# LasseWolter/laughter-detection-icsi

Hardware: AMD Instinct MI355X
Metric: 1 s@16 kHz segments/sec (featurize+ResNet fwd/bwd) (higher is better)
Workload: dtype f32 (64->64 and 32->32 convolutions: f16x2 split operands with per-tile power-of-two scales, f32 accumulate; error vs float64 within 1.5x of the exact-f32 kernels'); 1 GPU; BASELINE configs[2]: end-to-end featurize (HIP fbank 44 mel) + ResNetBigger resnet_base fwd/bwd + clip + Adam, random labels, dropout 0.5; global_batch=512, parallelism=dp1, overlap_wgrad=False, overlap_wgrad_small=True, bf16x3_convs=True, f16x2_convs=True, relu_bits=True, virtual_a1=True

## Files before the change

### include/lad_hip.h

```cpp
#ifndef LAD_HIP_H
#define LAD_HIP_H

#include <stdint.h>

#ifdef __cplusplus
extern "C" {
#endif

#define LAD_VERSION 100

enum lad_status {
    LAD_OK = 0,
    LAD_ERR_INVALID = -1,
    LAD_ERR_HIP = -2,
    LAD_ERR_NOMEM = -3,
    LAD_NOT_COVERED = 1
};

int lad_version(void);
const char *lad_last_error(void);

enum lad_pad_mode {
    LAD_PAD_KALDI_MIRROR = 0,
    LAD_PAD_CENTER_REFLECT = 1,
// ... 132 lines not shown

int lad_stem_fwd(const float *feat, const float *weight, float *out, float *stat_partials, int64_t batch, int32_t H,
                 int32_t W, int32_t cout, void *stream);
int lad_stem_fwd_eval(const float *feat, const float *weight, const float *scale, const float *shift, float *out,
                      int64_t batch, int32_t H, int32_t W, int32_t cout, int64_t frame_stride, int64_t frames_avail,
                      void *stream);
int64_t lad_stem_moments_workspace_doubles(void);
int64_t lad_stem_moments_doubles(void);
int lad_stem_bn_stats(const float *feat, const float *weight, const float *gamma, const float *beta, float *running_mean,
                      float *running_var, float momentum, float *coef, double *moments, double *workspace, int64_t batch, int32_t H,
                      int32_t W, int32_t cout, void *stream);
int64_t lad_stem_bwd_onepass_workspace_floats(void);
int lad_stem_bwd_onepass(const float *feat, const float *weight, const float *dy, const float *coef, const float *gamma,
                         const double *moments, float *workspace, float *dw, float *dgamma, float *dbeta, int64_t batch, int32_t H,
                         int32_t W, int32_t cout, void *stream);
int64_t lad_stem_wgrad_workspace_floats(void);
int lad_stem_wgrad(const float *feat, const float *dout, float *workspace, float *dw, int64_t batch, int32_t H,
                   int32_t W, int32_t cout, void *stream);
int lad_stem_wgrad_bn(const float *feat, const float *dy, const float *x, const float *weight, const float *coef,
                      const float *bcoef, float *workspace, float *dw, int64_t batch, int32_t H, int32_t W, int32_t cout,
                      void *stream);
int64_t lad_stem_bn_bwd_groups(int64_t batch, int32_t H, int32_t W);
int lad_stem_bn_bwd_sums(const float *feat, const float *weight, const float *dy, const float *coef, float *partials,
                         int64_t batch, int32_t H, int32_t W, int32_t cout, void *stream);

int lad_bn_finalize(float *stat_partials, int64_t n_tiles, int32_t channels, int64_t count, const float *gamma,
                    const float *beta, float *running_mean, float *running_var, float momentum, float *coef,
                    void *stream);
int lad_bn_finalize_pair(float *stat_partials_a, float *stat_partials_b, int64_t n_tiles, int32_t channels, int64_t count,
                         const float *gamma_a, const float *beta_a, float *running_mean_a, float *running_var_a, float *coef_a,
                         const float *gamma_b, const float *beta_b, float *running_mean_b, float *running_var_b, float *coef_b,
                         float momentum, void *stream);
int lad_bn_act(const float *x, const float *coef, const float *res, const float *res_coef, float *y, int64_t batch,
               int32_t H, int32_t W, int32_t channels, int32_t relu, void *stream);
int64_t lad_bn_bwd_workspace_floats(int32_t channels);
int lad_bn_bwd(const float *dy, const float *y, const float *x, const float *coef, const float *gamma,
               const float *xs, const float *scoef, const float *sgamma, float *dx, float *aux, float *dgamma,
               float *dbeta, float *dsgamma, float *dsbeta, float *workspace, float *bcoef, float *pre_partials,
               int64_t pre_tiles, int64_t batch, int32_t H, int32_t W, int32_t channels, int32_t relu, int32_t mode,
               void *stream);
int lad_bn_act_bits(const float *x, const float *coef, const float *res, const float *res_coef, float *y,
                    uint64_t *y_bits, int64_t batch, int32_t H, int32_t W, int32_t channels, void *stream);
int lad_bn_bwd_bits(const float *dy, const uint64_t *y_bits, const float *x, const float *coef, const float *gamma,
                    float *dx, float *dgamma, float *dbeta, float *workspace, float *bcoef, float *pre_partials,
                    int64_t pre_tiles, int64_t batch, int32_t H, int32_t W, int32_t channels, void *stream);
int lad_conv_fwd_bnstat(const float *in, const float *wt, const float *addend, float *out, float *stat_partials,
                        const float *bn_x, const float *bn_y, const float *bn_coef, int64_t batch, int32_t H, int32_t W,
                        int32_t cin, int32_t cout, int32_t taps, void *stream);

int lad_pool_fwd(const float *x, float *pooled, int64_t batch, int32_t H, int32_t W, int32_t channels, void *stream);
int lad_pool_bwd(const float *dpooled, float *dx, int64_t batch, int32_t H, int32_t W, int32_t channels, void *stream);
int64_t lad_head_workspace_floats(int64_t batch, int32_t F);
int lad_head_fwd_train(const float *const *params, const float *pooled, int64_t batch, int32_t F, const float *drop1,
                       const float *drop2, const int32_t *labels, float momentum, float *h, float *stats,
                       float *probs, float *metrics, void *stream);
int lad_head_fwd_train_rng(const float *const *params, const float *pooled, int64_t batch, int32_t F, float *drop1, float *drop2, float keep,
                           uint64_t seed, int64_t *rng_counter, int64_t *nbt, int32_t n_nbt, const int32_t *labels, float momentum,
// ... 63 lines not shown
```

### laughter-detection-icsi_amd/_hip.py

```python
import ctypes
import os

import torch

_HERE = os.path.dirname(os.path.abspath(__file__))
LIB_PATH = os.environ.get("LAD_HIP_LIB") or os.path.join(_HERE, "liblad_hip.so")

c_void_p = ctypes.c_void_p
c_int = ctypes.c_int
c_i64 = ctypes.c_int64
c_float = ctypes.c_float
c_double = ctypes.c_double
c_i32 = ctypes.c_int32
c_float_p = ctypes.POINTER(ctypes.c_float)


class LadHipError(RuntimeError):
    pass


class FbankCfg(ctypes.Structure):
    _fields_ = [("n_fft", ctypes.c_int32), ("frame_len", ctypes.c_int32), ("hop", ctypes.c_int32),
                ("n_mels", ctypes.c_int32), ("n_mfcc", ctypes.c_int32), ("pad_mode", ctypes.c_int32),
                ("log_mode", ctypes.c_int32), ("remove_dc", ctypes.c_int32), ("preemph", ctypes.c_float),
# ... 67 lines not shown
    "lad_conv_wgrad": (c_int, [c_void_p] * 5 + [c_i64, c_i32, c_i32, c_i32, c_i32, c_i32, c_void_p]),
    "lad_stem_fwd": (c_int, [c_void_p] * 4 + [c_i64, c_i32, c_i32, c_i32, c_void_p]),
    "lad_stem_fwd_eval": (c_int, [c_void_p] * 5 + [c_i64, c_i32, c_i32, c_i32, c_i64, c_i64, c_void_p]),
    "lad_stem_wgrad_workspace_floats": (c_i64, []),
    "lad_stem_wgrad": (c_int, [c_void_p] * 4 + [c_i64, c_i32, c_i32, c_i32, c_void_p]),
    "lad_stem_wgrad_bn": (c_int, [c_void_p] * 8 + [c_i64, c_i32, c_i32, c_i32, c_void_p]),
    "lad_stem_bn_bwd_groups": (c_i64, [c_i64, c_i32, c_i32]),
    "lad_stem_bn_bwd_sums": (c_int, [c_void_p] * 5 + [c_i64, c_i32, c_i32, c_i32, c_void_p]),
    "lad_bn_finalize": (c_int, [c_void_p, c_i64, c_i32, c_i64, c_void_p, c_void_p, c_void_p, c_void_p, c_float,
                                c_void_p, c_void_p]),
    "lad_stem_moments_workspace_doubles": (c_i64, []),
    "lad_stem_moments_doubles": (c_i64, []),
    "lad_stem_bn_stats": (c_int, [c_void_p] * 6 + [c_float] + [c_void_p] * 3 + [c_i64, c_i32, c_i32, c_i32, c_void_p]),
    "lad_stem_bwd_onepass_workspace_floats": (c_i64, []),
    "lad_stem_bwd_onepass": (c_int, [c_void_p] * 10 + [c_i64, c_i32, c_i32, c_i32, c_void_p]),
    "lad_bn_finalize_pair": (c_int, [c_void_p, c_void_p, c_i64, c_i32, c_i64] + [c_void_p] * 10 + [c_float, c_void_p]),
    "lad_bn_act": (c_int, [c_void_p] * 5 + [c_i64, c_i32, c_i32, c_i32, c_i32, c_void_p]),
    "lad_bn_bwd_workspace_floats": (c_i64, [c_i32]),
    "lad_bn_act_bits": (c_int, [c_void_p] * 6 + [c_i64, c_i32, c_i32, c_i32, c_void_p]),
    "lad_bn_bwd_bits": (c_int, [c_void_p] * 11 + [c_i64, c_i64, c_i32, c_i32, c_i32, c_void_p]),
    "lad_bn_bwd": (c_int, [c_void_p] * 17 + [c_i64, c_i64, c_i32, c_i32, c_i32, c_i32, c_i32, c_void_p]),
    "lad_conv_fwd_bnstat": (c_int, [c_void_p] * 8 + [c_i64, c_i32, c_i32, c_i32, c_i32, c_i32, c_void_p]),
    "lad_pool_fwd": (c_int, [c_void_p, c_void_p, c_i64, c_i32, c_i32, c_i32, c_void_p]),
    "lad_pool_bwd": (c_int, [c_void_p, c_void_p, c_i64, c_i32, c_i32, c_i32, c_void_p]),
    "lad_head_workspace_floats": (c_i64, [c_i64, c_i32]),
    "lad_head_fwd_train": (c_int, [c_void_p, c_void_p, c_i64, c_i32, c_void_p, c_void_p, c_void_p, c_float,
                                   c_void_p, c_void_p, c_void_p, c_void_p, c_void_p]),
    "lad_head_fwd_train_rng": (c_int, [c_void_p, c_void_p, c_i64, c_i32, c_void_p, c_void_p, c_float, ctypes.c_uint64, c_void_p, c_void_p, c_i32,
                                       c_void_p, c_float, c_void_p, c_void_p, c_void_p, c_void_p, c_void_p]),
    "lad_head_fwd_eval": (c_int, [c_void_p, c_void_p, c_i64, c_i32, c_void_p, c_void_p]),
    "lad_bce_metrics": (c_int, [c_void_p, c_void_p, c_i64, c_void_p, c_void_p]),
    "lad_head_bwd": (c_int, [c_void_p] * 7 + [c_i64, c_i32] + [c_void_p] * 6),
    "lad_f16_packed_weight_halfs": (c_i64, [c_i32, c_i32, c_i32]),
    "lad_f16_pack_weights": (c_int, [c_void_p, c_i32, c_i32, c_i32, c_void_p, c_void_p]),
# ... 67 lines not shown
```

### laughter-detection-icsi_amd/csrc/bn.hip

```cpp
#include "lad_common.h"
#include "lad_device.h"
#include "lad_bn_math.h"

namespace {
using namespace lad;

constexpr float BN_EPS = 1e-5f;
constexpr int THREADS = 256;

struct FinSet {
    const float *partials, *gamma, *beta;
    float *running_mean, *running_var, *coef;
};
struct FinSets {
    FinSet s[2];
};
__global__ void bn_finalize_kernel(FinSets sets, int64_t n_tiles, int C, double count, float momentum) {
    const FinSet f = sets.s[blockIdx.y];
    const float *__restrict__ partials = f.partials;
    float *__restrict__ coef = f.coef;
    const int c = blockIdx.x;
    double s1 = 0.0, s2 = 0.0;
    int64_t t = threadIdx.x;
    const int64_t bd = blockDim.x;
// ... 218 lines not shown
                    const float4 rr = res[idx];
                    o.x += rr.x; o.y += rr.y; o.z += rr.z; o.w += rr.w;
                } else if (RES == 2) {
                    const float4 rr = res[idx];
                    o.x += fmaf(rr.x, rs.x, rh.x); o.y += fmaf(rr.y, rs.y, rh.y);
                    o.z += fmaf(rr.z, rs.z, rh.z); o.w += fmaf(rr.w, rs.w, rh.w);
                }
                if (relu) {
                    o.x = fmaxf(o.x, 0.f); o.y = fmaxf(o.y, 0.f); o.z = fmaxf(o.z, 0.f); o.w = fmaxf(o.w, 0.f);
                }
            }
            y[idx] = o;
            if (BITS) {
                const unsigned long long word = pack_sign_bits(o, threadIdx.x & 63);
                if ((threadIdx.x & 15) == 0) bits[idx >> 4] = word;
            }
        }
    }
}

template <int C, bool SHORT>
__global__ __launch_bounds__(THREADS) void bn_bwd_reduce_kernel(const float4 *__restrict__ dy, const float4 *__restrict__ y,
                                                                const float4 *__restrict__ x, const float *__restrict__ coef,
                                                                const float4 *__restrict__ xs, const float *__restrict__ scoef,
                                                                float *__restrict__ partials, int64_t rows, int relu,
                                                                const unsigned long long *__restrict__ bits) {
    constexpr int C4 = C / 4;
    constexpr int RP = THREADS / C4;
    constexpr int K = SHORT ? 3 : 2;
    const int c4 = threadIdx.x % C4, rp = threadIdx.x / C4;
// ... 285 lines not shown
}
}

extern "C" int lad_bn_act(const float *x, const float *coef, const float *res, const float *res_coef, float *y,
                          int64_t batch, int32_t H, int32_t W, int32_t channels, int32_t relu, void *stream) {
    return bn_act_impl(x, coef, res, res_coef, y, nullptr, batch, H, W, channels, relu, stream, "lad_bn_act");
}

extern "C" int lad_bn_act_bits(const float *x, const float *coef, const float *res, const float *res_coef, float *y,
                               uint64_t *y_bits, int64_t batch, int32_t H, int32_t W, int32_t channels, void *stream) {
    using namespace lad;
    LAD_REQUIRE(y_bits, "lad_bn_act_bits: null sign-bit buffer");
    return bn_act_impl(x, coef, res, res_coef, y, (unsigned long long *)y_bits, batch, H, W, channels, 1, stream, "lad_bn_act_bits");
}

extern "C" int64_t lad_bn_bwd_workspace_floats(int32_t channels) { return (int64_t)BWD_GROUPS * 3 * channels; }

namespace {
int bn_bwd_impl(const float *dy, const float *y, const unsigned long long *bits, const float *x, const float *coef, const float *gamma,
                const float *xs, const float *scoef, const float *sgamma, float *dx, float *aux,
                float *dgamma, float *dbeta, float *dsgamma, float *dsbeta, float *workspace, float *bcoef,
                float *pre_partials, int64_t pre_tiles, int64_t batch, int32_t H, int32_t W, int32_t channels,
                int32_t relu, int32_t mode, void *stream) {
    using namespace lad;
    LAD_REQUIRE(relu != 3 || (bits && channels == 64), "lad_bn_bwd_bits: sign bits are kept for 64-channel activations only");
    LAD_REQUIRE(dy && coef && gamma && dgamma && dbeta && workspace && bcoef, "lad_bn_bwd: null buffer");
    LAD_REQUIRE(x || (pre_partials && !dx), "lad_bn_bwd: x may only be omitted when the sums are given and nothing is applied");
    LAD_REQUIRE(dx || mode == 0, "lad_bn_bwd: dx may only be omitted (sums and coefficients only) in mode 0");
    LAD_REQUIRE(relu >= 0 && relu <= 3, "lad_bn_bwd: relu must be 0 (none), 1 (mask from y), 2 (mask recomputed from x) or 3 (sign bits: lad_bn_bwd_bits)");
    LAD_REQUIRE(relu != 1 || y, "lad_bn_bwd: relu = 1 needs y");
// ... 82 lines not shown
```

### laughter-detection-icsi_amd/csrc/lad_stem_taps.h

```cpp
#pragma once
#include "lad_device.h"

namespace lad {

constexpr int STEM_TM = 128;
constexpr int TAPW = 12;
__device__ __forceinline__ void fill_taps(const float *__restrict__ feat, const Geom &g, int H, int W, int64_t q0,
                                          int64_t frame_stride, int64_t frames_avail, float *tap_s ) {
    const int r = threadIdx.x;
    if (r < STEM_TM) {
        const int64_t q = q0 + r;
        float v[9];
#pragma unroll
        for (int t = 0; t < 9; ++t) v[t] = 0.0f;
        float flag = 0.0f;
        if (q < g.body) {
            const int64_t b = q / g.img;
            const int rr = (int)(q - b * g.img);
            const int yp = rr / g.Wp, xp = rr - yp * g.Wp;
            if (yp >= 1 && xp >= 1) {
                flag = 1.0f;
                const int y = yp - 1, x = xp - 1;
                const int64_t f0 = b * frame_stride;
#pragma unroll
                for (int ky = 0; ky < 3; ++ky)
#pragma unroll
                    for (int kx = 0; kx < 3; ++kx) {
                        const int yy = y + ky - 1, xx = x + kx - 1;
                        const bool ok = yy >= 0 && yy < H && xx >= 0 && xx < W && (f0 + yy) < frames_avail;
                        v[ky * 3 + kx] = ok ? feat[(f0 + yy) * W + xx] : 0.0f;
                    }
            }
        }
        float4 *dst = reinterpret_cast<float4 *>(tap_s + r * TAPW);
        dst[0] = make_float4(v[0], v[1], v[2], v[3]);
        dst[1] = make_float4(v[4], v[5], v[6], v[7]);
        dst[2] = make_float4(v[8], flag, 0.f, 0.f);
    }
}
__device__ __forceinline__ bool read_taps(const float *tap_s, int r, float (&v)[9]) {
    const float4 *src = reinterpret_cast<const float4 *>(tap_s + r * TAPW);
    const float4 a = src[0], b = src[1], c = src[2];
    v[0] = a.x; v[1] = a.y; v[2] = a.z; v[3] = a.w; v[4] = b.x; v[5] = b.y; v[6] = b.z; v[7] = b.w; v[8] = c.x;
    return c.y != 0.0f;
}


}
```

### laughter-detection-icsi_amd/csrc/stem.hip

```cpp
#include "lad_common.h"
#include "lad_device.h"
#include "lad_stem_taps.h"
#include "lad_bn_math.h"

namespace {
using namespace lad;

constexpr int THREADS = 256;
constexpr int TM = lad::STEM_TM;
constexpr int COUT = 64;
constexpr int CQ = COUT / 4;
constexpr int RL = THREADS / CQ;
constexpr int MAX_GROUPS = 1536;

template <bool STORE>
__global__ __launch_bounds__(THREADS) void stem_fwd_kernel(const float *__restrict__ feat, const float *__restrict__ w ,
                                                           float *__restrict__ out, float *__restrict__ partials, Geom g,
                                                           int H, int W) {
    const int tid = threadIdx.x, cq = tid % CQ, rl = tid / CQ;
    float wr[4][9];
#pragma unroll
    for (int c = 0; c < 4; ++c)
#pragma unroll
        for (int t = 0; t < 9; ++t) wr[c][t] = w[(cq * 4 + c) * 9 + t];
// ... 34 lines not shown
            const int k = tid / COUT, c = tid - k * COUT;
            float s = 0.f;
#pragma unroll
            for (int p = 0; p < RL; ++p) s += red[p][k][c];
            partials[((int64_t)blockIdx.x * 2 + k) * COUT + c] = s;
        }
    }
}

__global__ __launch_bounds__(THREADS) void stem_fwd_eval_kernel(const float *__restrict__ feat, const float *__restrict__ w,
                                                                const float *__restrict__ scale, const float *__restrict__ shift,
                                                                float *__restrict__ out, Geom g, int H, int W,
                                                                int64_t frame_stride, int64_t frames_avail) {
    const int tid = threadIdx.x, cq = tid % CQ, rl = tid / CQ;
    float wr[4][9];
#pragma unroll
    for (int c = 0; c < 4; ++c)
#pragma unroll
        for (int t = 0; t < 9; ++t) wr[c][t] = w[(cq * 4 + c) * 9 + t];
    const float4 sc = *reinterpret_cast<const float4 *>(scale + cq * 4);
    const float4 sh = *reinterpret_cast<const float4 *>(shift + cq * 4);
    const int64_t q0 = (int64_t)blockIdx.x * TM;
    __shared__ __attribute__((aligned(16))) float tap_s[TM * TAPW];
    fill_taps(feat, g, H, W, q0, frame_stride, frames_avail, tap_s);
    __syncthreads();
    for (int r = rl; r < TM; r += RL) {
        const int64_t q = q0 + r;
        if (q >= g.rows) break;
        float4 o = make_float4(0.f, 0.f, 0.f, 0.f);
        float v[9];
        if (read_taps(tap_s, r, v)) {
            float acc[4] = {0, 0, 0, 0};
#pragma unroll
            for (int t = 0; t < 9; ++t)
#pragma unroll
                for (int c = 0; c < 4; ++c) acc[c] = fmaf(v[t], wr[c][t], acc[c]);
            o = make_float4(fmaxf(fmaf(acc[0], sc.x, sh.x), 0.f), fmaxf(fmaf(acc[1], sc.y, sh.y), 0.f),
                            fmaxf(fmaf(acc[2], sc.z, sh.z), 0.f), fmaxf(fmaf(acc[3], sc.w, sh.w), 0.f));
        }
        *reinterpret_cast<float4 *>(out + q * COUT + cq * 4) = o;
    }
}

template <int MODE>
__global__ __launch_bounds__(THREADS) void stem_wgrad_kernel(const float *__restrict__ feat, const float *__restrict__ dout,
                                                             const float *__restrict__ x, const float *__restrict__ w,
                                                             const float *__restrict__ coef,
                                                             const float *__restrict__ bcoef, float *__restrict__ slabs,
                                                             Geom g, int H, int W, int64_t n_tiles) {
    const int tid = threadIdx.x, cq = tid % CQ, rl = tid / CQ;
    float acc[4][9];
#pragma unroll
    for (int c = 0; c < 4; ++c)
#pragma unroll
// ... 288 lines not shown
        coef[0 * COUT + c] = scale;
        coef[1 * COUT + c] = beta[c] - (float)mean * scale;
        coef[2 * COUT + c] = (float)mean;
        coef[3 * COUT + c] = invstd;
        coef[4 * COUT + c] = (float)(mean - (double)(float)mean);
        coef[5 * COUT + c] = (float)(invstd_d - (double)invstd);
        if (running_mean != nullptr) {
            const double unbiased = count > 1.0 ? var * count / (count - 1.0) : var;
            running_mean[c] = (1.0f - momentum) * running_mean[c] + momentum * (float)mean;
            running_var[c] = (1.0f - momentum) * running_var[c] + momentum * (float)unbiased;
        }
    }
}

constexpr int BWD1_COLS = COUT * 9 + 2 * COUT;
__global__ __launch_bounds__(THREADS) void stem_bwd_onepass_kernel(const float *__restrict__ feat, const float *__restrict__ w,
                                                                   const float *__restrict__ dy, const float *__restrict__ coef,
                                                                   const double *__restrict__ mom, float *__restrict__ slabs, Geom g, int H,
                                                                   int W, int64_t n_tiles) {
    const int tid = threadIdx.x, cq = tid % CQ, rl = tid / CQ;
    float acc[4][9];
#pragma unroll
    for (int c = 0; c < 4; ++c)
#pragma unroll
        for (int t = 0; t < 9; ++t) acc[c][t] = 0.f;
    float wr[4][9];
#pragma unroll
    for (int c = 0; c < 4; ++c)
#pragma unroll
        for (int t = 0; t < 9; ++t) wr[c][t] = w[(cq * 4 + c) * 9 + t];
    const float4 fsc = *reinterpret_cast<const float4 *>(coef + cq * 4);
    const float4 fsh = *reinterpret_cast<const float4 *>(coef + COUT + cq * 4);
    const Norm4 nm = load_norm(coef, COUT, cq * 4);
    const float m = (float)mom[MOM_N];
    float4 a0 = make_float4(0.f, 0.f, 0.f, 0.f), a1 = a0;
    __shared__ __attribute__((aligned(16))) float tap_s[TM * TAPW];
    constexpr int NR = TM / RL;
    for (int64_t tile = blockIdx.x; tile < n_tiles; tile += gridDim.x) {
        const int64_t q0 = tile * TM;
        float4 dv[NR];
#pragma unroll
        for (int k = 0; k < NR; ++k) {
            const int64_t q = q0 + rl + k * RL;
            dv[k] = q < g.rows ? *reinterpret_cast<const float4 *>(dy + q * COUT + cq * 4) : make_float4(0.f, 0.f, 0.f, 0.f);
        }
        __syncthreads();
        fill_taps(feat, g, H, W, q0, H, (int64_t)1 << 62, tap_s);
        __syncthreads();
#pragma unroll
        for (int k = 0; k < NR; ++k) {
            const int r = rl + k * RL;
            const int64_t q = q0 + r;
            if (q >= g.rows) break;
            float v[9];
            if (read_taps(tap_s, r, v)) {
                float xa[4] = {0, 0, 0, 0};
#pragma unroll
                for (int t = 0; t < 9; ++t)
#pragma unroll
                    for (int c = 0; c < 4; ++c) xa[c] = fmaf(v[t], wr[c][t], xa[c]);
                const float4 xv = make_float4(xa[0], xa[1], xa[2], xa[3]);
                const float4 d = mask_from_x(dv[k], xv, fsc, fsh);
                const float4 xh = xhat4(xv, nm);
                a0.x += d.x; a0.y += d.y; a0.z += d.z; a0.w += d.w;
                a1.x = fmaf(d.x, xh.x, a1.x); a1.y = fmaf(d.y, xh.y, a1.y); a1.z = fmaf(d.z, xh.z, a1.z); a1.w = fmaf(d.w, xh.w, a1.w);
                const float dd[4] = {d.x, d.y, d.z, d.w};
#pragma unroll
                for (int t = 0; t < 9; ++t) {
                    const float gt = v[t] - m;
#pragma unroll
                    for (int c = 0; c < 4; ++c) acc[c][t] = fmaf(gt, dd[c], acc[c][t]);
                }
            }
        }
    }
    __shared__ float red[RL][BWD1_COLS];
#pragma unroll
    for (int c = 0; c < 4; ++c)
#pragma unroll
        for (int t = 0; t < 9; ++t) red[rl][(cq * 4 + c) * 9 + t] = acc[c][t];
    *reinterpret_cast<float4 *>(&red[rl][COUT * 9 + cq * 4]) = a0;
    *reinterpret_cast<float4 *>(&red[rl][COUT * 10 + cq * 4]) = a1;
    __syncthreads();
    for (int e = tid; e < BWD1_COLS; e += THREADS) {
        float sacc = 0.f;
#pragma unroll
        for (int p = 0; p < RL; ++p) sacc += red[p][e];
        slabs[(int64_t)blockIdx.x * BWD1_COLS + e] = sacc;
// ... 159 lines not shown
    LAD_REQUIRE(cout == COUT && batch >= 1 && H >= 1 && W >= 1, "lad_stem_bn_stats: bad arguments");
    const int groups = (int)std::min<int64_t>(MOM_GROUPS, batch);
    const size_t lds = std::max<size_t>((size_t)(H + 2) * (W + 2) * sizeof(float), (size_t)18 * MOM_THREADS * sizeof(double));
    LAD_REQUIRE(lds <= 60 * 1024, "lad_stem_bn_stats: an image of %d x %d does not fit the workgroup's LDS", H, W);
    hipStream_t st = (hipStream_t)stream;
    hipLaunchKernelGGL(stem_moments_kernel, dim3(groups), dim3(MOM_THREADS), lds, st, feat, workspace, batch, H, W);
    int rc = check_launch("stem_moments_kernel");
    if (rc) return rc;
    hipLaunchKernelGGL(stem_stats_finalize_kernel, dim3(1), dim3(MOMF_THREADS), 0, st, (const double *)workspace, groups, weight,
                       (double)(batch * (int64_t)H * W), gamma, beta, running_mean, running_var, momentum, coef, moments);
    return check_launch("stem_stats_finalize_kernel");
}

extern "C" int64_t lad_stem_bwd_onepass_workspace_floats(void) { return (int64_t)(MAX_GROUPS + 1) * BWD1_COLS; }

extern "C" int lad_stem_bwd_onepass(const float *feat, const float *weight, const float *dy, const float *coef, const float *gamma,
                                    const double *moments, float *workspace, float *dw, float *dgamma, float *dbeta, int64_t batch,
                                    int32_t H, int32_t W, int32_t cout, void *stream) {
    using namespace lad;
    LAD_REQUIRE(feat && weight && dy && coef && gamma && moments && workspace && dw && dgamma && dbeta, "lad_stem_bwd_onepass: null buffer");
    LAD_REQUIRE(cout == COUT && batch >= 1 && H >= 1 && W >= 1, "lad_stem_bwd_onepass: bad arguments");
    const Geom g = make_geom(batch, H, W);
    const int64_t n_tiles = ceil_div(g.rows, TM);
    const int groups = (int)std::min<int64_t>(MAX_GROUPS, n_tiles);
    hipStream_t st = (hipStream_t)stream;
    float *sums = workspace + (int64_t)MAX_GROUPS * BWD1_COLS;
    hipLaunchKernelGGL(stem_bwd_onepass_kernel, dim3(groups), dim3(THREADS), 0, st, feat, weight, dy, coef, moments, workspace, g, H, W, n_tiles);
    int rc = check_launch("stem_bwd_onepass_kernel");
    if (rc) return rc;
    unsigned int *ticket = launch_ticket();
    LAD_REQUIRE(ticket, "lad_stem_bwd_onepass: no ticket");
    static_assert(BWD1_COLS <= 64 * CS_PARTS, "the last workgroup takes a column per thread");
    hipLaunchKernelGGL(stem_bwd_finish_kernel, dim3((unsigned)ceil_div(BWD1_COLS, 64)), dim3(64 * CS_PARTS), 0, st, (const float *)workspace, sums,
                       groups, moments, weight, coef, gamma, dw, dgamma, dbeta, ticket);
    return check_launch("stem_bwd_finish_kernel");
}
```

### laughter-detection-icsi_amd/engine.py

```python
import ctypes
import math

import torch

import _hip

_VP = ctypes.c_void_p


PREDICT_CHUNK = {"fp16": 8192, "fp32": 2048}
BASE_WIDTHS = (64, 32, 16, 16)
STREAM_SUPER_MAX = 1 << 20


class _LazyLevels(dict):

    def __init__(self, make):
        super().__init__()
        self._make = make

    def __missing__(self, key):
        value = self[key] = self._make(key)
        return value

# ... 17 lines not shown
class _BnSpec:
    def __init__(self, name, c):
        self.name, self.c = name, c
        self.g = self.b = self.rm = self.rv = self.gg = self.gb = None
        self.coef = None


class _BlockSpec:
    def __init__(self, name):
        self.name = name
        self.conv1 = self.bn1 = self.conv2 = self.bn2 = self.sc_conv = self.sc_bn = None


class ResNetEngine:
    KERNEL_OPTIONS = ("bf16x3", "bf16x3_32", "f16x2", "f16x2_32", "relu_bits", "virtual_a1", "fuse_bn_bwd", "fuse_bn_bwd_b3", "fuse_bn_bwd_wgrad", "fuse_s2_shortcut",
                      "fuse_s2_shortcut_wgrad", "s2_b3")

    def __init__(self, model):
        self.model = model
        self.device = None
        self._flat_p = self._flat_g = None
        self._plans = {}
        self._step_count = 0
        self._lib = None
        self._grad_dirty = False
        self._train_forwards = 0
        self._fold_tag = None
        self._weights_version = 0
        self.fuse_bn_bwd = False
        self.overlap_wgrad = False
        self.overlap_wgrad_small = "auto"
        self.stem_onepass = True
        self.bf16x3 = True
        self.fuse_bn_bwd_b3 = True
        self.fuse_bn_bwd_wgrad = True
        self.f16x2 = True
        self.f16x2_32 = True
        self.bf16x3_32 = True
        self.virtual_a1 = True
        self.s2_b3 = True
        self.stream_direct = True
        self.stream_level2 = True
        self.strip_block_fused = True
        self.small_block_fused = True
        self.stream_super = True
        self.tail_fused = True
        self.strip2_resident = True
# ... 502 lines not shown
                else:
                    _hip.check(lib.lad_conv_b3c_fwd_f32_bnrelu(_hip.ptr(a["c1"]), _hip.ptr(a["coef1"]), _hip.ptr(b.conv2.wt3_f),
                                                               _hip.ptr(b.conv2.b), _hip.ptr(a["c2"]), _hip.ptr(part), B, ho, wo, b.conv2.cin, st),
                               "lad_conv_b3c_fwd_f32_bnrelu " + b.conv2.name)
                self._mark_end(label, t0)
            else:
                self._bn_act(a["c1"], a["coef1"], None, None, a["a1"], B, ho, wo, co)
                self._conv(b.conv2, a["a1"], a["c2"], part, B)
            self._bn_coef(b.bn2, a["coef2"], part, B, ho, wo, train)
            if b.sc_conv is not None:
                if not fuse_sc_fwd:
                    self._conv(b.sc_conv, cur, a["cs"], part, B)
                    self._bn_coef(b.sc_bn, a["coefs"], part, B, ho, wo, train)
                self._bn_act(a["c2"], a["coef2"], a["cs"], a["coefs"], a["y"], B, ho, wo, co)
            elif self._use_bits(b, a):
                _hip.check(lib.lad_bn_act_bits(_hip.ptr(a["c2"]), _hip.ptr(a["coef2"]), _hip.ptr(cur), None, _hip.ptr(a["y"]),
                                               _hip.ptr(a["ybits"]), B, ho, wo, co, st), "lad_bn_act_bits")
                a["bits_live"] = True
            else:
                self._bn_act(a["c2"], a["coef2"], cur, None, a["y"], B, ho, wo, co)
                a["bits_live"] = False
            a["x"] = cur
            cur = a["y"]
        last = blocks[-1].conv2
        _hip.check(lib.lad_pool_fwd(_hip.ptr(cur), _hip.ptr(p["pooled"]), B, p["h4"], p["w4"], last.cout, st), "lad_pool_fwd")
        if True:
            m1 = m2 = None
            rng = isinstance(drop_masks, str) and drop_masks == "rng"
            if drop_masks is not None and not rng:
                m1, m2 = drop_masks
                _hip.require_cuda(m1, "drop mask 1", torch.float32)
                _hip.require_cuda(m2, "drop mask 2", torch.float32)
# ... 845 lines not shown
                    _hip.check(lib.lad_conv_s2_dgrad_fused(_hip.ptr(dc1), _hip.ptr(c1s.wt_d), _hip.ptr(aux), _hip.ptr(sc.wt_d), _hip.ptr(dx),
                                                           B, hi, wi, c1s.cin, c1s.cout, st), "lad_conv_s2_dgrad_fused " + c1s.name)
                else:
                    _hip.check(lib.lad_conv_s2_dgrad(_hip.ptr(dc1), _hip.ptr(c1s.wt_d), _hip.ptr(dx), B, hi, wi, c1s.cin, c1s.cout, 9, 0,
                                                     st), "lad_conv_s2_dgrad " + c1s.name)
                if not fuse_sc:
                    self._on_side(lambda sst, sc=sc, aux=aux, xin=a["x"]: _hip.check(lib.lad_conv_s2_wgrad(
                        _hip.ptr(xin), _hip.ptr(aux), _hip.ptr(self._wg_ws(p, sc)), _hip.ptr(sc.gw), None, B, hi, wi, sc.cin, sc.cout, 1,
                        sst), "lad_conv_s2_wgrad " + sc.name), aux, small=sc.cin <= 32)
                if not self.fuse_s2_shortcut:
                    _hip.check(lib.lad_conv_s2_dgrad(_hip.ptr(aux), _hip.ptr(sc.wt_d), _hip.ptr(dx), B, hi, wi, sc.cin, sc.cout, 1, 1, st),
                               "lad_conv_s2_dgrad " + sc.name)
                dy = dx
        if p.get("stem_mom_live"):
            bn = self.stem_bn
            _hip.check(lib.lad_stem_bwd_onepass(_hip.ptr(x), _hip.ptr(self.stem_w), _hip.ptr(dy), _hip.ptr(p["stem_coef"]), _hip.ptr(bn.g),
                                                _hip.ptr(p["stem_mom"]), _hip.ptr(p["stem_bwd_ws"]), _hip.ptr(self.stem_gw), _hip.ptr(bn.gg),
                                                _hip.ptr(bn.gb), B, H, W, self.stem_cout, st), "lad_stem_bwd_onepass")
        else:
            groups = int(lib.lad_stem_bn_bwd_groups(B, H, W))
            _hip.check(lib.lad_stem_bn_bwd_sums(_hip.ptr(x), _hip.ptr(self.stem_w), _hip.ptr(dy), _hip.ptr(p["stem_coef"]),
                                                _hip.ptr(p["partials"]), B, H, W, self.stem_cout, st), "lad_stem_bn_bwd_sums")
            bn = self.stem_bn
            _hip.check(lib.lad_bn_bwd(_hip.ptr(dy), None, None, _hip.ptr(p["stem_coef"]), _hip.ptr(bn.g), None, None, None, None,
                                      None, _hip.ptr(bn.gg), _hip.ptr(bn.gb), None, None, _hip.ptr(p["bn_ws"]), _hip.ptr(p["bcoef"]),
                                      _hip.ptr(p["partials"]), groups, B, H, W, bn.c, 2, 0, st), "lad_bn_bwd " + bn.name)
            self._on_side(lambda sst: _hip.check(lib.lad_stem_wgrad_bn(_hip.ptr(x), _hip.ptr(dy), None, _hip.ptr(self.stem_w),
                                                                       _hip.ptr(p["stem_coef"]), _hip.ptr(p["bcoef"]),
                                                                       _hip.ptr(p["wgrad_ws"]), _hip.ptr(self.stem_gw), B, H, W,
                                                                       self.stem_cout, sst), "lad_stem_wgrad_bn"), dy)
        if self._defer_on:
            self._defer_on = False
            self._join_side()
# ... 115 lines not shown
```

Baseline: 47620 segments/s.

## Recompute stem residual in block bn_act and prefetch next tile in stem backward

Adds a fused bn_act_bits kernel for the first residual block that recomputes the stem conv+BN+ReLU output from the input features and stem weights, instead of reading the stored stem activation. It also adds a variant of the one-pass stem backward kernel that double-buffers the tap tiles in shared memory and prefetches the next tile's taps and dy into registers while the current tile is computed. Both are on by default. The first trades extra FLOPs and LDS traffic for less global-memory reads. The second raises register and LDS use, which may lower occupancy.

```diff
diff --git a/include/lad_hip.h b/include/lad_hip.h
--- a/include/lad_hip.h
+++ b/include/lad_hip.h
@@ -170,6 +170,9 @@
 int lad_stem_bwd_onepass(const float *feat, const float *weight, const float *dy, const float *coef, const float *gamma,
                          const double *moments, float *workspace, float *dw, float *dgamma, float *dbeta, int64_t batch, int32_t H,
                          int32_t W, int32_t cout, void *stream);
+int lad_stem_bwd_onepass_variant(const float *feat, const float *weight, const float *dy, const float *coef, const float *gamma,
+                                 const double *moments, float *workspace, float *dw, float *dgamma, float *dbeta, int64_t batch,
+                                 int32_t H, int32_t W, int32_t cout, int32_t variant, void *stream);
 int64_t lad_stem_wgrad_workspace_floats(void);
 int lad_stem_wgrad(const float *feat, const float *dout, float *workspace, float *dw, int64_t batch, int32_t H,
                    int32_t W, int32_t cout, void *stream);
@@ -197,6 +200,8 @@
                void *stream);
 int lad_bn_act_bits(const float *x, const float *coef, const float *res, const float *res_coef, float *y,
                     uint64_t *y_bits, int64_t batch, int32_t H, int32_t W, int32_t channels, void *stream);
+int lad_bn_act_bits_stem(const float *x, const float *coef, const float *feat, const float *stem_weight, const float *stem_coef,
+                         float *y, uint64_t *y_bits, int64_t batch, int32_t H, int32_t W, int32_t channels, void *stream);
 int lad_bn_bwd_bits(const float *dy, const uint64_t *y_bits, const float *x, const float *coef, const float *gamma,
                     float *dx, float *dgamma, float *dbeta, float *workspace, float *bcoef, float *pre_partials,
                     int64_t pre_tiles, int64_t batch, int32_t H, int32_t W, int32_t channels, void *stream);
diff --git a/laughter-detection-icsi_amd/_hip.py b/laughter-detection-icsi_amd/_hip.py
--- a/laughter-detection-icsi_amd/_hip.py
+++ b/laughter-detection-icsi_amd/_hip.py
@@ -105,10 +105,12 @@
     "lad_stem_bn_stats": (c_int, [c_void_p] * 6 + [c_float] + [c_void_p] * 3 + [c_i64, c_i32, c_i32, c_i32, c_void_p]),
     "lad_stem_bwd_onepass_workspace_floats": (c_i64, []),
     "lad_stem_bwd_onepass": (c_int, [c_void_p] * 10 + [c_i64, c_i32, c_i32, c_i32, c_void_p]),
+    "lad_stem_bwd_onepass_variant": (c_int, [c_void_p] * 10 + [c_i64, c_i32, c_i32, c_i32, c_i32, c_void_p]),
     "lad_bn_finalize_pair": (c_int, [c_void_p, c_void_p, c_i64, c_i32, c_i64] + [c_void_p] * 10 + [c_float, c_void_p]),
     "lad_bn_act": (c_int, [c_void_p] * 5 + [c_i64, c_i32, c_i32, c_i32, c_i32, c_void_p]),
     "lad_bn_bwd_workspace_floats": (c_i64, [c_i32]),
     "lad_bn_act_bits": (c_int, [c_void_p] * 6 + [c_i64, c_i32, c_i32, c_i32, c_void_p]),
+    "lad_bn_act_bits_stem": (c_int, [c_void_p] * 7 + [c_i64, c_i32, c_i32, c_i32, c_void_p]),
     "lad_bn_bwd_bits": (c_int, [c_void_p] * 11 + [c_i64, c_i64, c_i32, c_i32, c_i32, c_void_p]),
     "lad_bn_bwd": (c_int, [c_void_p] * 17 + [c_i64, c_i64, c_i32, c_i32, c_i32, c_i32, c_i32, c_void_p]),
     "lad_conv_fwd_bnstat": (c_int, [c_void_p] * 8 + [c_i64, c_i32, c_i32, c_i32, c_i32, c_i32, c_void_p]),
diff --git a/laughter-detection-icsi_amd/csrc/bn.hip b/laughter-detection-icsi_amd/csrc/bn.hip
--- a/laughter-detection-icsi_amd/csrc/bn.hip
+++ b/laughter-detection-icsi_amd/csrc/bn.hip
@@ -1,6 +1,7 @@
 #include "lad_common.h"
 #include "lad_device.h"
 #include "lad_bn_math.h"
+#include "lad_stem_taps.h"
 
 namespace {
 using namespace lad;
@@ -256,6 +257,84 @@
             if (BITS) {
                 const unsigned long long word = pack_sign_bits(o, threadIdx.x & 63);
                 if ((threadIdx.x & 15) == 0) bits[idx >> 4] = word;
+            }
+        }
+    }
+}
+
+constexpr int STEM_RES_MAX_W = 128;
+constexpr int STEM_RES_NX = 3;
+__global__ __launch_bounds__(THREADS) void bn_act_stem_bits_kernel(const float4 *__restrict__ x, const float *__restrict__ coef,
+                                                                   const float *__restrict__ feat, const float *__restrict__ sw,
+                                                                   const float *__restrict__ scoef, float4 *__restrict__ y, RowGeom g,
+                                                                   int H, int W, unsigned long long *__restrict__ bits) {
+    constexpr int C = 64;
+    const int cq = threadIdx.x & 15, c = cq * 4;
+    const int per_row = g.Wp << 4;
+    const float4 sc = *reinterpret_cast<const float4 *>(coef + c);
+    const float4 sh = *reinterpret_cast<const float4 *>(coef + C + c);
+    const float4 ssc = *reinterpret_cast<const float4 *>(scoef + c);
+    const float4 ssh = *reinterpret_cast<const float4 *>(scoef + C + c);
+    __shared__ __attribute__((aligned(16))) float w_s[9][C];
+    for (int i = threadIdx.x; i < 9 * C; i += THREADS) w_s[i % 9][i / 9] = sw[i];
+    const int Wq = W + 2;
+    __shared__ float fr[3][STEM_RES_MAX_W + 2];
+    for (int64_t r = blockIdx.x; r < g.n_img_rows; r += gridDim.x) {
+        const int64_t b = r / g.Hp;
+        const int yp = (int)(r - b * g.Hp);
+        const bool border_row = (yp == 0);
+        const int64_t base = r * per_row;
+        float4 xv[STEM_RES_NX];
+#pragma unroll
+        for (int k = 0; k < STEM_RES_NX; ++k) {
+            const int f = (int)threadIdx.x + k * THREADS;
+            if (!border_row && f < per_row && (f >> 4) != 0) xv[k] = x[base + f];
+        }
+        __syncthreads();
+        if (!border_row) {
+            for (int i = threadIdx.x; i < 3 * Wq; i += THREADS) {
+                const int k = i / Wq, xx = i - k * Wq - 1, yy = yp - 2 + k;
+                fr[k][xx + 1] = (xx >= 0 && xx < W && yy >= 0 && yy < H) ? feat[(b * H + yy) * W + xx] : 0.0f;
+            }
+        }
+        __syncthreads();
+        for (int f0 = 0; f0 < per_row; f0 += STEM_RES_NX * THREADS) {
+            if (f0 > 0) {
+#pragma unroll
+                for (int k = 0; k < STEM_RES_NX; ++k) {
+                    const int f = f0 + (int)threadIdx.x + k * THREADS;
+                    if (!border_row && f < per_row) xv[k] = x[base + f];
+                }
+            }
+#pragma unroll
+            for (int k = 0; k < STEM_RES_NX; ++k) {
+                const int f = f0 + (int)threadIdx.x + k * THREADS;
+                if (f < per_row) {
+                    const int xp = f >> 4;
+                    float4 o = make_float4(0.f, 0.f, 0.f, 0.f);
+                    if (!(border_row | (xp == 0))) {
+                        float v[9];
+#pragma unroll
+                        for (int ky = 0; ky < 3; ++ky)
+#pragma unroll
+                            for (int kx = 0; kx < 3; ++kx) v[ky * 3 + kx] = fr[ky][xp - 1 + kx];
+                        asm volatile("" ::: "memory");
+                        float wr[4][9];
+#pragma unroll
+                        for (int t = 0; t < 9; ++t) {
+                            const float4 wq = *reinterpret_cast<const float4 *>(&w_s[t][c]);
+                            wr[0][t] = wq.x; wr[1][t] = wq.y; wr[2][t] = wq.z; wr[3][t] = wq.w;
+                        }
+                        const float4 rr = stem_act4(v, wr, ssc, ssh);
+                        const float4 v4 = xv[k];
+                        o = make_float4(fmaf(v4.x, sc.x, sh.x), fmaf(v4.y, sc.y, sh.y), fmaf(v4.z, sc.z, sh.z), fmaf(v4.w, sc.w, sh.w));
+                        o.x += rr.x; o.y += rr.y; o.z += rr.z; o.w += rr.w;
+                        o.x = fmaxf(o.x, 0.f); o.y = fmaxf(o.y, 0.f); o.z = fmaxf(o.z, 0.f); o.w = fmaxf(o.w, 0.f);
+                    }
+                    y[base + f] = o;
+                    const unsigned long long word = pack_sign_bits(o, threadIdx.x & 63);
+                    if ((threadIdx.x & 15) == 0) bits[(base + f) >> 4] = word;
+                }
             }
         }
     }
@@ -571,6 +650,20 @@
     return bn_act_impl(x, coef, res, res_coef, y, (unsigned long long *)y_bits, batch, H, W, channels, 1, stream, "lad_bn_act_bits");
 }
 
+extern "C" int lad_bn_act_bits_stem(const float *x, const float *coef, const float *feat, const float *stem_weight, const float *stem_coef,
+                                    float *y, uint64_t *y_bits, int64_t batch, int32_t H, int32_t W, int32_t channels, void *stream) {
+    using namespace lad;
+    LAD_REQUIRE(x && coef && feat && stem_weight && stem_coef && y && y_bits, "lad_bn_act_bits_stem: null buffer");
+    LAD_REQUIRE(channels == 64, "lad_bn_act_bits_stem: the stem has 64 channels (got %d)", channels);
+    LAD_REQUIRE(batch >= 0 && H >= 1 && W >= 1 && W <= STEM_RES_MAX_W, "lad_bn_act_bits_stem: bad geometry (W must be 1..%d)", STEM_RES_MAX_W);
+    if (batch == 0) return LAD_OK;
+    const RowGeom g = make_row_geom(batch, H, W);
+    const unsigned grid = (unsigned)std::min<int64_t>(g.n_img_rows, 256 * 256);
+    hipLaunchKernelGGL(bn_act_stem_bits_kernel, dim3(grid), dim3(THREADS), 0, (hipStream_t)stream, (const float4 *)x, coef, feat, stem_weight,
+                       stem_coef, (float4 *)y, g, H, W, (unsigned long long *)y_bits);
+    return check_launch("bn_act_stem_bits_kernel");
+}
+
 extern "C" int64_t lad_bn_bwd_workspace_floats(int32_t channels) { return (int64_t)BWD_GROUPS * 3 * channels; }
 
 namespace {
diff --git a/laughter-detection-icsi_amd/csrc/lad_stem_taps.h b/laughter-detection-icsi_amd/csrc/lad_stem_taps.h
--- a/laughter-detection-icsi_amd/csrc/lad_stem_taps.h
+++ b/laughter-detection-icsi_amd/csrc/lad_stem_taps.h
@@ -5,15 +5,14 @@
 
 constexpr int STEM_TM = 128;
 constexpr int TAPW = 12;
-__device__ __forceinline__ void fill_taps(const float *__restrict__ feat, const Geom &g, int H, int W, int64_t q0,
-                                          int64_t frame_stride, int64_t frames_avail, float *tap_s ) {
+__device__ __forceinline__ void gather_taps(const float *__restrict__ feat, const Geom &g, int H, int W, int64_t q0, int64_t frame_stride,
+                                            int64_t frames_avail, float (&v)[9], float &flag) {
     const int r = threadIdx.x;
+#pragma unroll
+    for (int t = 0; t < 9; ++t) v[t] = 0.0f;
+    flag = 0.0f;
     if (r < STEM_TM) {
         const int64_t q = q0 + r;
-        float v[9];
-#pragma unroll
-        for (int t = 0; t < 9; ++t) v[t] = 0.0f;
-        float flag = 0.0f;
         if (q < g.body) {
             const int64_t b = q / g.img;
             const int rr = (int)(q - b * g.img);
@@ -32,11 +31,22 @@
                     }
             }
         }
+    }
+}
+__device__ __forceinline__ void store_taps(const float (&v)[9], float flag, float *tap_s ) {
+    const int r = threadIdx.x;
+    if (r < STEM_TM) {
         float4 *dst = reinterpret_cast<float4 *>(tap_s + r * TAPW);
         dst[0] = make_float4(v[0], v[1], v[2], v[3]);
         dst[1] = make_float4(v[4], v[5], v[6], v[7]);
         dst[2] = make_float4(v[8], flag, 0.f, 0.f);
     }
+}
+__device__ __forceinline__ void fill_taps(const float *__restrict__ feat, const Geom &g, int H, int W, int64_t q0,
+                                          int64_t frame_stride, int64_t frames_avail, float *tap_s ) {
+    float v[9], flag;
+    gather_taps(feat, g, H, W, q0, frame_stride, frames_avail, v, flag);
+    store_taps(v, flag, tap_s);
 }
 __device__ __forceinline__ bool read_taps(const float *tap_s, int r, float (&v)[9]) {
     const float4 *src = reinterpret_cast<const float4 *>(tap_s + r * TAPW);
@@ -45,5 +55,21 @@
     return c.y != 0.0f;
 }
 
+__device__ __forceinline__ void load_stem_weights(const float *__restrict__ w , int cq, float (&wr)[4][9]) {
+#pragma unroll
+    for (int c = 0; c < 4; ++c)
+#pragma unroll
+        for (int t = 0; t < 9; ++t) wr[c][t] = w[(cq * 4 + c) * 9 + t];
+}
+__device__ __forceinline__ float4 stem_act4(const float (&v)[9], const float (&wr)[4][9], float4 sc, float4 sh) {
+    float acc[4] = {0, 0, 0, 0};
+#pragma unroll
+    for (int t = 0; t < 9; ++t)
+#pragma unroll
+        for (int c = 0; c < 4; ++c) acc[c] = fmaf(v[t], wr[c][t], acc[c]);
+    return make_float4(fmaxf(fmaf(acc[0], sc.x, sh.x), 0.f), fmaxf(fmaf(acc[1], sc.y, sh.y), 0.f),
+                       fmaxf(fmaf(acc[2], sc.z, sh.z), 0.f), fmaxf(fmaf(acc[3], sc.w, sh.w), 0.f));
+}
+
 
 }
diff --git a/laughter-detection-icsi_amd/csrc/stem.hip b/laughter-detection-icsi_amd/csrc/stem.hip
--- a/laughter-detection-icsi_amd/csrc/stem.hip
+++ b/laughter-detection-icsi_amd/csrc/stem.hip
@@ -72,10 +72,7 @@
                                                                 int64_t frame_stride, int64_t frames_avail) {
     const int tid = threadIdx.x, cq = tid % CQ, rl = tid / CQ;
     float wr[4][9];
-#pragma unroll
-    for (int c = 0; c < 4; ++c)
-#pragma unroll
-        for (int t = 0; t < 9; ++t) wr[c][t] = w[(cq * 4 + c) * 9 + t];
+    load_stem_weights(w, cq, wr);
     const float4 sc = *reinterpret_cast<const float4 *>(scale + cq * 4);
     const float4 sh = *reinterpret_cast<const float4 *>(shift + cq * 4);
     const int64_t q0 = (int64_t)blockIdx.x * TM;
@@ -87,15 +84,7 @@
         if (q >= g.rows) break;
         float4 o = make_float4(0.f, 0.f, 0.f, 0.f);
         float v[9];
-        if (read_taps(tap_s, r, v)) {
-            float acc[4] = {0, 0, 0, 0};
-#pragma unroll
-            for (int t = 0; t < 9; ++t)
-#pragma unroll
-                for (int c = 0; c < 4; ++c) acc[c] = fmaf(v[t], wr[c][t], acc[c]);
-            o = make_float4(fmaxf(fmaf(acc[0], sc.x, sh.x), 0.f), fmaxf(fmaf(acc[1], sc.y, sh.y), 0.f),
-                            fmaxf(fmaf(acc[2], sc.z, sh.z), 0.f), fmaxf(fmaf(acc[3], sc.w, sh.w), 0.f));
-        }
+        if (read_taps(tap_s, r, v)) o = stem_act4(v, wr, sc, sh);
         *reinterpret_cast<float4 *>(out + q * COUT + cq * 4) = o;
     }
 }
@@ -414,6 +403,7 @@
 }
 
 constexpr int BWD1_COLS = COUT * 9 + 2 * COUT;
+template <bool AHEAD>
 __global__ __launch_bounds__(THREADS) void stem_bwd_onepass_kernel(const float *__restrict__ feat, const float *__restrict__ w,
                                                                    const float *__restrict__ dy, const float *__restrict__ coef,
                                                                    const double *__restrict__ mom, float *__restrict__ slabs, Geom g, int H,
@@ -434,26 +424,47 @@
     const Norm4 nm = load_norm(coef, COUT, cq * 4);
     const float m = (float)mom[MOM_N];
     float4 a0 = make_float4(0.f, 0.f, 0.f, 0.f), a1 = a0;
-    __shared__ __attribute__((aligned(16))) float tap_s[TM * TAPW];
+    __shared__ __attribute__((aligned(16))) float tap_s[2][TM * TAPW];
     constexpr int NR = TM / RL;
+    auto load_dy = [&](int64_t t, float4 (&d)[NR]) {
+#pragma unroll
+        for (int k = 0; k < NR; ++k) {
+            const int64_t q = t * TM + rl + k * RL;
+            d[k] = q < g.rows ? *reinterpret_cast<const float4 *>(dy + q * COUT + cq * 4) : make_float4(0.f, 0.f, 0.f, 0.f);
+        }
+    };
+    float4 dv[NR];
+    int slot = 0;
+    if (AHEAD && (int64_t)blockIdx.x < n_tiles) {
+        float tv[9], tf;
+        gather_taps(feat, g, H, W, (int64_t)blockIdx.x * TM, H, (int64_t)1 << 62, tv, tf);
+        load_dy(blockIdx.x, dv);
+        store_taps(tv, tf, tap_s[0]);
+    }
     for (int64_t tile = blockIdx.x; tile < n_tiles; tile += gridDim.x) {
-        const int64_t q0 = tile * TM;
-        float4 dv[NR];
-#pragma unroll
-        for (int k = 0; k < NR; ++k) {
-            const int64_t q = q0 + rl + k * RL;
-            dv[k] = q < g.rows ? *reinterpret_cast<const float4 *>(dy + q * COUT + cq * 4) : make_float4(0.f, 0.f, 0.f, 0.f);
-        }
-        __syncthreads();
-        fill_taps(feat, g, H, W, q0, H, (int64_t)1 << 62, tap_s);
-        __syncthreads();
+        const int64_t q0 = tile * TM, next = tile + gridDim.x;
+        float tv[9], tf;
+        float4 dn[NR];
+        if (AHEAD) {
+            __syncthreads();
+            if (next < n_tiles) {
+                gather_taps(feat, g, H, W, next * TM, H, (int64_t)1 << 62, tv, tf);
+                load_dy(next, dn);
+            }
+        } else {
+            load_dy(tile, dv);
+            __syncthreads();
+            fill_taps(feat, g, H, W, q0, H, (int64_t)1 << 62, tap_s[0]);
+            __syncthreads();
+        }
+        const float *tcur = tap_s[slot];
 #pragma unroll
         for (int k = 0; k < NR; ++k) {
             const int r = rl + k * RL;
             const int64_t q = q0 + r;
             if (q >= g.rows) break;
             float v[9];
-            if (read_taps(tap_s, r, v)) {
+            if (read_taps(tcur, r, v)) {
                 float xa[4] = {0, 0, 0, 0};
 #pragma unroll
                 for (int t = 0; t < 9; ++t)
@@ -472,6 +483,14 @@
                     for (int c = 0; c < 4; ++c) acc[c][t] = fmaf(gt, dd[c], acc[c][t]);
                 }
             }
+        }
+        if (AHEAD) {
+            if (next < n_tiles) {
+                store_taps(tv, tf, tap_s[slot ^ 1]);
+#pragma unroll
+                for (int k = 0; k < NR; ++k) dv[k] = dn[k];
+            }
+            slot ^= 1;
         }
     }
     __shared__ float red[RL][BWD1_COLS];
@@ -661,18 +680,25 @@
 
 extern "C" int64_t lad_stem_bwd_onepass_workspace_floats(void) { return (int64_t)(MAX_GROUPS + 1) * BWD1_COLS; }
 
-extern "C" int lad_stem_bwd_onepass(const float *feat, const float *weight, const float *dy, const float *coef, const float *gamma,
-                                    const double *moments, float *workspace, float *dw, float *dgamma, float *dbeta, int64_t batch,
-                                    int32_t H, int32_t W, int32_t cout, void *stream) {
+extern "C" int lad_stem_bwd_onepass_variant(const float *feat, const float *weight, const float *dy, const float *coef, const float *gamma,
+                                            const double *moments, float *workspace, float *dw, float *dgamma, float *dbeta, int64_t batch,
+                                            int32_t H, int32_t W, int32_t cout, int32_t variant, void *stream) {
     using namespace lad;
     LAD_REQUIRE(feat && weight && dy && coef && gamma && moments && workspace && dw && dgamma && dbeta, "lad_stem_bwd_onepass: null buffer");
     LAD_REQUIRE(cout == COUT && batch >= 1 && H >= 1 && W >= 1, "lad_stem_bwd_onepass: bad arguments");
+    LAD_REQUIRE(variant == 0 || variant == 1, "lad_stem_bwd_onepass_variant: variant must be 0 or 1 (got %d)", variant);
+    const bool ahead = variant == 1;
     const Geom g = make_geom(batch, H, W);
     const int64_t n_tiles = ceil_div(g.rows, TM);
     const int groups = (int)std::min<int64_t>(MAX_GROUPS, n_tiles);
     hipStream_t st = (hipStream_t)stream;
     float *sums = workspace + (int64_t)MAX_GROUPS * BWD1_COLS;
-    hipLaunchKernelGGL(stem_bwd_onepass_kernel, dim3(groups), dim3(THREADS), 0, st, feat, weight, dy, coef, moments, workspace, g, H, W, n_tiles);
+    if (ahead)
+        hipLaunchKernelGGL(stem_bwd_onepass_kernel<true>, dim3(groups), dim3(THREADS), 0, st, feat, weight, dy, coef, moments, workspace, g, H, W,
+                           n_tiles);
+    else
+        hipLaunchKernelGGL(stem_bwd_onepass_kernel<false>, dim3(groups), dim3(THREADS), 0, st, feat, weight, dy, coef, moments, workspace, g, H, W,
+                           n_tiles);
     int rc = check_launch("stem_bwd_onepass_kernel");
     if (rc) return rc;
     unsigned int *ticket = launch_ticket();
@@ -682,3 +708,9 @@
                        groups, moments, weight, coef, gamma, dw, dgamma, dbeta, ticket);
     return check_launch("stem_bwd_finish_kernel");
 }
+
+extern "C" int lad_stem_bwd_onepass(const float *feat, const float *weight, const float *dy, const float *coef, const float *gamma,
+                                    const double *moments, float *workspace, float *dw, float *dgamma, float *dbeta, int64_t batch,
+                                    int32_t H, int32_t W, int32_t cout, void *stream) {
+    return lad_stem_bwd_onepass_variant(feat, weight, dy, coef, gamma, moments, workspace, dw, dgamma, dbeta, batch, H, W, cout, 1, stream);
+}
diff --git a/laughter-detection-icsi_amd/engine.py b/laughter-detection-icsi_amd/engine.py
--- a/laughter-detection-icsi_amd/engine.py
+++ b/laughter-detection-icsi_amd/engine.py
@@ -55,7 +55,7 @@
 
 class ResNetEngine:
     KERNEL_OPTIONS = ("bf16x3", "bf16x3_32", "f16x2", "f16x2_32", "relu_bits", "virtual_a1", "fuse_bn_bwd", "fuse_bn_bwd_b3", "fuse_bn_bwd_wgrad", "fuse_s2_shortcut",
-                      "fuse_s2_shortcut_wgrad", "s2_b3")
+                      "fuse_s2_shortcut_wgrad", "s2_b3", "stem_residual_recompute", "stem_bwd_ahead")
 
     def __init__(self, model):
         self.model = model
@@ -72,6 +72,8 @@
         self.overlap_wgrad = False
         self.overlap_wgrad_small = "auto"
         self.stem_onepass = True
+        self.stem_residual_recompute = True
+        self.stem_bwd_ahead = True
         self.bf16x3 = True
         self.fuse_bn_bwd_b3 = True
         self.fuse_bn_bwd_wgrad = True
@@ -604,8 +606,13 @@
                     self._bn_coef(b.sc_bn, a["coefs"], part, B, ho, wo, train)
                 self._bn_act(a["c2"], a["coef2"], a["cs"], a["coefs"], a["y"], B, ho, wo, co)
             elif self._use_bits(b, a):
-                _hip.check(lib.lad_bn_act_bits(_hip.ptr(a["c2"]), _hip.ptr(a["coef2"]), _hip.ptr(cur), None, _hip.ptr(a["y"]),
-                                               _hip.ptr(a["ybits"]), B, ho, wo, co, st), "lad_bn_act_bits")
+                if self.stem_residual_recompute and self.stem_onepass and cur is p["stem_a"]:
+                    _hip.check(lib.lad_bn_act_bits_stem(_hip.ptr(a["c2"]), _hip.ptr(a["coef2"]), _hip.ptr(x), _hip.ptr(self.stem_w),
+                                                        _hip.ptr(p["stem_coef"]), _hip.ptr(a["y"]), _hip.ptr(a["ybits"]), B, ho, wo, co, st),
+                               "lad_bn_act_bits_stem")
+                else:
+                    _hip.check(lib.lad_bn_act_bits(_hip.ptr(a["c2"]), _hip.ptr(a["coef2"]), _hip.ptr(cur), None, _hip.ptr(a["y"]),
+                                                   _hip.ptr(a["ybits"]), B, ho, wo, co, st), "lad_bn_act_bits")
                 a["bits_live"] = True
             else:
                 self._bn_act(a["c2"], a["coef2"], cur, None, a["y"], B, ho, wo, co)
@@ -1481,9 +1488,10 @@
                 dy = dx
         if p.get("stem_mom_live"):
             bn = self.stem_bn
-            _hip.check(lib.lad_stem_bwd_onepass(_hip.ptr(x), _hip.ptr(self.stem_w), _hip.ptr(dy), _hip.ptr(p["stem_coef"]), _hip.ptr(bn.g),
-                                                _hip.ptr(p["stem_mom"]), _hip.ptr(p["stem_bwd_ws"]), _hip.ptr(self.stem_gw), _hip.ptr(bn.gg),
-                                                _hip.ptr(bn.gb), B, H, W, self.stem_cout, st), "lad_stem_bwd_onepass")
+            _hip.check(lib.lad_stem_bwd_onepass_variant(_hip.ptr(x), _hip.ptr(self.stem_w), _hip.ptr(dy), _hip.ptr(p["stem_coef"]), _hip.ptr(bn.g),
+                                                        _hip.ptr(p["stem_mom"]), _hip.ptr(p["stem_bwd_ws"]), _hip.ptr(self.stem_gw), _hip.ptr(bn.gg),
+                                                        _hip.ptr(bn.gb), B, H, W, self.stem_cout, 1 if self.stem_bwd_ahead else 0, st),
+                       "lad_stem_bwd_onepass")
         else:
             groups = int(lib.lad_stem_bn_bwd_groups(B, H, W))
             _hip.check(lib.lad_stem_bn_bwd_sums(_hip.ptr(x), _hip.ptr(self.stem_w), _hip.ptr(dy), _hip.ptr(p["stem_coef"]),
```

Result: no change. 47940 segments/s, median of 6 (+0.7%).
